# martinsbruveris/tensorflow-image-models

Hardware: NVIDIA H100
Metric: images/sec fwd bs=256 224px (higher is better)
Workload: dtype bf16

## Files before the change

tensorflow-image-models_b200/csrc/gemm_epilogue.cuh:

```cuda
#pragma once
#include "common.cuh"

namespace tfimm {

struct GemmParams {
  int M, N, K;
  const float* bias;
  const float* gamma;
  int act;
  int has_res;
  int act_post;
  void* c;
  const void* res;
  long ldc, ldr;
  const float* a_scale;
  int a_rows_per_img, a_imgs;
  int conv;
  int cv_cblocks;
  int cv_ks, cv_stride, cv_pad;
  int cv_pb, cv_ph, cv_pw;
  int cv_tiles_x, cv_tiles_y;
  int cv_B, cv_Ho, cv_Wo;
  int tk_imgs, m_out, glu;
  long img_c, img_r;
  const void* mul;
  long ld_mul, img_mul;
};

__device__ __forceinline__ long epilogue_row_offset(const GemmParams& p, int m_blk, int r, long ld) {
  if (p.conv == 0) {
    const long m = (long)m_blk * 128 + r;
    return m < p.M ? m * ld : -1;
  }
  const int tx = m_blk % p.cv_tiles_x, tyb = m_blk / p.cv_tiles_x;
  const int ty = tyb % p.cv_tiles_y, tb = tyb / p.cv_tiles_y;
  const int per_img = p.cv_ph * p.cv_pw;
  const int b = tb * p.cv_pb + r / per_img;
  const int y = ty * p.cv_ph + (r % per_img) / p.cv_pw;
  const int x = tx * p.cv_pw + r % p.cv_pw;
  if (b >= p.cv_B || y >= p.cv_Ho || x >= p.cv_Wo) return -1;
  return (((long)b * p.cv_Ho + y) * p.cv_Wo + x) * p.N;
}

template <int NP, bool kSharedRcp = false>
__device__ __forceinline__ void apply_act_pairs(uint64_t (&v)[NP], int act) {
  static_assert(NP % 2 == 0, "activations are evaluated on groups of four elements");
  switch (act) {
    case kActGelu:
#pragma unroll
      for (int j = 0; j < NP; j += 2) {
        gelu4<kSharedRcp>(v[j], v[j + 1]);
      }
      break;
    case kActSwish:
#pragma unroll
      for (int j = 0; j < NP; j += 2) {
        swish4<kSharedRcp>(v[j], v[j + 1]);
      }
      break;
    case kActNone:
      break;
    default:
#pragma unroll
      for (int j = 0; j < NP; ++j) {
        float a, b;
        unpack2(v[j], a, b);
        v[j] = pack2(apply_act<false>(a, act), apply_act<false>(b, act));
      }
      break;
  }
}

__device__ __forceinline__ uint64_t ld_pair_or(const float* __restrict__ vec, int n, int N, float neutral) {
  if (n + 1 < N) {
    const float2 f = __ldg(reinterpret_cast<const float2*>(vec + n));
    return pack2(f.x, f.y);
  }
  return pack2(n < N ? __ldg(vec + n) : neutral, neutral);
}

__device__ __forceinline__ uint64_t ld_out_pair(const float* p, bool two) {
  if (two) {
    const float2 f = *reinterpret_cast<const float2*>(p);
    return pack2(f.x, f.y);
  }
  return pack2(*p, 0.f);
}
__device__ __forceinline__ uint64_t ld_out_pair(const __nv_bfloat16* p, bool two) {
  if (two) {
    const float2 f = unpack_bf16x2(*reinterpret_cast<const uint32_t*>(p));
    return pack2(f.x, f.y);
  }
  return pack2(__bfloat162float(*p), 0.f);
}
__device__ __forceinline__ void st_out_pair(float* p, uint64_t v, bool two) {
  float a, b;
  unpack2(v, a, b);
  if (two) *reinterpret_cast<float2*>(p) = make_float2(a, b);
  else *p = a;
}
__device__ __forceinline__ void st_out_pair(__nv_bfloat16* p, uint64_t v, bool two) {
  float a, b;
  unpack2(v, a, b);
  if (two) *reinterpret_cast<uint32_t*>(p) = pack_bf16x2(a, b);
  else *p = __float2bfloat16_rn(a);
}

template <typename OutT, int BN>
__device__ __forceinline__ void epilogue_frag(const GemmParams& p, float (&acc)[BN / 2], int m_blk, int n_blk,
                                              int wg_row0) {
  constexpr int kRun = BN >= 256 ? 2 : 4;
  const int lane = threadIdx.x & 31, wq = (threadIdx.x >> 5) & 3;
  const int r = wg_row0 + wq * 16 + (lane >> 2);
  const long off_c[2] = {epilogue_row_offset(p, m_blk, r, p.ldc), epilogue_row_offset(p, m_blk, r + 8, p.ldc)};
  const long off_r[2] = {p.has_res ? epilogue_row_offset(p, m_blk, r, p.ldr) : -1,
                         p.has_res ? epilogue_row_offset(p, m_blk, r + 8, p.ldr) : -1};
  OutT* __restrict__ C = reinterpret_cast<OutT*>(p.c);
  const OutT* R = reinterpret_cast<const OutT*>(p.res);
#pragma unroll
  for (int g0 = 0; g0 < BN / 8; g0 += kRun) {
    if (n_blk * BN + g0 * 8 >= p.N) break;
    uint64_t b[kRun], s[kRun], res[kRun][2];
#pragma unroll
    for (int j = 0; j < kRun; ++j) {
      const int n = n_blk * BN + (g0 + j) * 8 + 2 * (lane & 3);
      const bool in = n < p.N, two = n + 1 < p.N;
      b[j] = p.bias != nullptr ? ld_pair_or(p.bias, n, p.N, 0.f) : 0;
      s[j] = p.gamma != nullptr ? ld_pair_or(p.gamma, n, p.N, 1.f) : 0;
#pragma unroll
      for (int h = 0; h < 2; ++h)
        res[j][h] = p.has_res && in && off_r[h] >= 0 ? ld_out_pair(R + off_r[h] + n, two) : 0;
    }
#pragma unroll
    for (int j = 0; j < kRun; ++j) {
      const int g = g0 + j;
      const int n = n_blk * BN + g * 8 + 2 * (lane & 3);
      if (n_blk * BN + g * 8 >= p.N) break;
      const bool in = n < p.N, two = n + 1 < p.N;
      uint64_t v[2] = {pack2(acc[4 * g + 0], acc[4 * g + 1]), pack2(acc[4 * g + 2], acc[4 * g + 3])};
      if (p.bias != nullptr) {
        v[0] = add2(v[0], b[j]);
        v[1] = add2(v[1], b[j]);
      }
      if (!p.act_post) apply_act_pairs(v, p.act);
      if (p.gamma != nullptr) {
        v[0] = mul2(v[0], s[j]);
        v[1] = mul2(v[1], s[j]);
      }
      if (p.has_res) {
#pragma unroll
        for (int h = 0; h < 2; ++h)
          if (in && off_r[h] >= 0) v[h] = add2(v[h], res[j][h]);
      }
      if (p.act_post) apply_act_pairs(v, p.act);
#pragma unroll
      for (int h = 0; h < 2; ++h)
        if (in && off_c[h] >= 0) st_out_pair(C + off_c[h] + n, v[h], two);
    }
  }
}

template <typename OutT>
constexpr int staged_chunk_cols() { return 128 / (int)sizeof(OutT); }
constexpr int kStagedBoxBytes = 64 * 128;

template <typename OutT>
__device__ __forceinline__ uint32_t staged_addr(uint32_t s_wg, int row, int col) {
  constexpr int kCols = staged_chunk_cols<OutT>();
  const uint32_t byte = (uint32_t)(col % kCols) * (uint32_t)sizeof(OutT);
  return s_wg + (uint32_t)(col / kCols) * kStagedBoxBytes + (uint32_t)row * 128u +
         ((((byte >> 4) ^ (uint32_t)(row & 7)) << 4) | (byte & 15u));
}
__device__ __forceinline__ uint64_t ld_staged_pair(const float*, uint32_t a) {
  float x, y;
  asm volatile("ld.shared.v2.f32 {%0, %1}, [%2];" : "=f"(x), "=f"(y) : "r"(a) : "memory");
  return pack2(x, y);
}
__device__ __forceinline__ uint64_t ld_staged_pair(const __nv_bfloat16*, uint32_t a) {
  uint32_t u;
  asm volatile("ld.shared.b32 %0, [%1];" : "=r"(u) : "r"(a) : "memory");
  const float2 f = unpack_bf16x2(u);
  return pack2(f.x, f.y);
}
__device__ __forceinline__ void st_staged_pair(float*, uint32_t a, uint64_t v) {
  float x, y;
  unpack2(v, x, y);
  asm volatile("st.shared.v2.f32 [%0], {%1, %2};" ::"r"(a), "f"(x), "f"(y) : "memory");
}
__device__ __forceinline__ void st_staged_pair(__nv_bfloat16*, uint32_t a, uint64_t v) {
  float x, y;
  unpack2(v, x, y);
  asm volatile("st.shared.b32 [%0], %1;" ::"r"(a), "r"(pack_bf16x2(x, y)) : "memory");
}

template <typename OutT, int BN>
__device__ __forceinline__ void epilogue_staged(const GemmParams& p, float (&acc)[BN / 2], int m_blk, int n_blk, int wg,
                                                uint32_t s_out, const float* s_bias, const float* s_gamma,
                                                uint32_t res_bar, const CUtensorMap* tmap_c) {
  constexpr int kCols = staged_chunk_cols<OutT>(), kChunks = BN / kCols;
  const int lane = threadIdx.x & 31, wq = (threadIdx.x >> 5) & 3;
  const int r = wq * 16 + (lane >> 2);
  const uint32_t s_wg = s_out + (uint32_t)(wg * kChunks * kStagedBoxBytes);
  OutT* const tag = nullptr;
  named_bar_sync<1>(256);
  if (p.has_res) mbar_wait(res_bar, 0);
#pragma unroll
  for (int g = 0; g < BN / 8; ++g) {
    const int c = g * 8 + 2 * (lane & 3);
    const uint32_t a0 = staged_addr<OutT>(s_wg, r, c), a1 = a0 + 8 * 128;
    uint64_t v[2] = {pack2(acc[4 * g + 0], acc[4 * g + 1]), pack2(acc[4 * g + 2], acc[4 * g + 3])};
    if (p.bias != nullptr) {
      const float2 b = *reinterpret_cast<const float2*>(s_bias + c);
      v[0] = add2(v[0], pack2(b.x, b.y));
      v[1] = add2(v[1], pack2(b.x, b.y));
    }
    if (!p.act_post) apply_act_pairs(v, p.act);
    if (p.gamma != nullptr) {
      const float2 s = *reinterpret_cast<const float2*>(s_gamma + c);
      v[0] = mul2(v[0], pack2(s.x, s.y));
      v[1] = mul2(v[1], pack2(s.x, s.y));
    }
    if (p.has_res) {
      v[0] = add2(v[0], ld_staged_pair(tag, a0));
      v[1] = add2(v[1], ld_staged_pair(tag, a1));
    }
    if (p.act_post) apply_act_pairs(v, p.act);
    st_staged_pair(tag, a0, v[0]);
    st_staged_pair(tag, a1, v[1]);
  }
  fence_proxy_async_smem();
  if (wg == 0) named_bar_sync<2>(128);
  else named_bar_sync<3>(128);
  const int row0 = m_blk * 128 + wg * 64;
  if ((threadIdx.x & 127) == 0 && row0 < p.M) {
#pragma unroll
    for (int ch = 0; ch < kChunks; ++ch) {
      const int col0 = n_blk * BN + ch * kCols;
      if (col0 < p.N) tma_store_2d(tmap_c, s_wg + (uint32_t)(ch * kStagedBoxBytes), col0, row0);
    }
    tma_store_commit();
    tma_store_wait_read<0>();
  }
}

template <typename OutT, int BN>
__device__ __forceinline__ void epilogue_token(const GemmParams& p, float (&acc)[BN / 2], int img, int m_blk, int n_blk,
                                               int wg_row0) {
  const int lane = threadIdx.x & 31, wq = (threadIdx.x >> 5) & 3;
  const int m0 = m_blk * 128 + wg_row0 + wq * 16 + (lane >> 2);
  const float b0 = p.bias != nullptr && m0 < p.M ? __ldg(p.bias + m0) : 0.f;
  const float b1 = p.bias != nullptr && m0 + 8 < p.M ? __ldg(p.bias + m0 + 8) : 0.f;
  const int rows[2] = {p.glu ? (m0 >> 4) * 8 + (m0 & 7) : m0, p.glu ? -1 : m0 + 8};
  OutT* __restrict__ C = reinterpret_cast<OutT*>(p.c) + (long)img * p.img_c;
  const OutT* R = reinterpret_cast<const OutT*>(p.res) + (long)img * p.img_r;
  const OutT* U = reinterpret_cast<const OutT*>(p.mul) + (long)img * p.img_mul;
#pragma unroll
  for (int g = 0; g < BN / 8; ++g) {
    const int n = n_blk * BN + g * 8 + 2 * (lane & 3);
    if (n_blk * BN + g * 8 >= p.N) break;
    const bool in = n < p.N, two = n + 1 < p.N;
    uint64_t v[2] = {pack2(acc[4 * g + 0] + b0, acc[4 * g + 1] + b0), pack2(acc[4 * g + 2] + b1, acc[4 * g + 3] + b1)};
    if (p.glu) {
      float x0, x1, g0, g1;
      unpack2(v[0], x0, x1);
      unpack2(v[1], g0, g1);
      v[0] = pack2(x0 * apply_act<false>(g0, p.act), x1 * apply_act<false>(g1, p.act));
    } else {
      apply_act_pairs(v, p.act);
    }
    if (p.gamma != nullptr) {
      const uint64_t s = ld_pair_or(p.gamma, n, p.N, 1.f);
      v[0] = mul2(v[0], s);
      v[1] = mul2(v[1], s);
    }
#pragma unroll
    for (int h = 0; h < 2; ++h) {
      const int row = rows[h];
      if (!in || row < 0 || row >= p.m_out) continue;
      if (p.mul != nullptr) v[h] = mul2(v[h], ld_out_pair(U + (long)row * p.ld_mul + n, two));
      if (p.has_res) v[h] = add2(v[h], ld_out_pair(R + (long)row * p.ldr + n, two));
      st_out_pair(C + (long)row * p.ldc + n, v[h], two);
    }
  }
}

template <typename OutT, int BN>
__device__ __forceinline__ void epilogue_glu_cols(const GemmParams& p, float (&acc)[BN / 2], int m_blk, int n_blk,
                                                  int wg_row0) {
  const int lane = threadIdx.x & 31, wq = (threadIdx.x >> 5) & 3;
  const int r = wg_row0 + wq * 16 + (lane >> 2);
  const long off_c[2] = {epilogue_row_offset(p, m_blk, r, p.ldc), epilogue_row_offset(p, m_blk, r + 8, p.ldc)};
  OutT* __restrict__ C = reinterpret_cast<OutT*>(p.c);
#pragma unroll
  for (int g = 0; g < BN / 8; ++g) {
    const int n = n_blk * BN + g * 8 + 2 * (lane & 3);
    if (n_blk * BN + g * 8 >= p.N) break;
    if (n >= p.N) continue;
    float bx = 0.f, bg = 0.f;
    if (p.bias != nullptr) {
      const float2 b = __ldg(reinterpret_cast<const float2*>(p.bias + n));
      bx = b.x; bg = b.y;
    }
#pragma unroll
    for (int h = 0; h < 2; ++h) {
      if (off_c[h] < 0) continue;
      const float x = acc[4 * g + 2 * h] + bx, gt = acc[4 * g + 2 * h + 1] + bg;
      const float y = x * apply_act<false>(gt, p.act);
      if constexpr (sizeof(OutT) == 2) C[off_c[h] + n / 2] = __float2bfloat16_rn(y);
      else C[off_c[h] + n / 2] = y;
    }
  }
}

}
```

tensorflow-image-models_b200/csrc/gemm_sm90.cu:

```cuda
#include <type_traits>

#include "gemm_epilogue.cuh"
#include "wgmma.cuh"

namespace tfimm {

namespace {

constexpr int kBlockM = 128;
constexpr int kRowBytes = 128;
constexpr int kConsumerThreads = 256;
constexpr int kProducerWarp = kConsumerThreads / 32;
constexpr int kNumGateWarps = 4;

enum ATransform : int {
  kANone = 0,
  kAGate = 1,
  kATf32 = 2,
};
enum GemmMode : int { kModeGemm = 0, kModeToken = 1, kModeGluCols = 2 };

template <int AX>
using OperandT = std::conditional_t<AX == kATf32, float, __nv_bfloat16>;
template <int AX>
constexpr int block_k() { return kRowBytes / (int)sizeof(OperandT<AX>); }
template <int AX>
constexpr int dtype_code() { return AX == kATf32 ? kF32 : kBF16; }

template <int BLOCK_N, typename OutT = float, bool STAGED = false>
struct GemmCfg {
  static constexpr int kABytes = kBlockM * kRowBytes;
  static constexpr int kBBytes = BLOCK_N * kRowBytes;
  static constexpr int kStageBytes = kABytes + kBBytes;
  static constexpr int kStages = STAGED && BLOCK_N == 64 ? 3 : 4;
  static constexpr int kOutBytes = STAGED ? kBlockM * BLOCK_N * (int)sizeof(OutT) : 0;
  static constexpr int kVecBytes = STAGED ? 2 * BLOCK_N * 4 : 0;
  static constexpr int kNumBarriers = 3 * kStages + 1;
  static constexpr int kSmemBytes =
      kStages * kStageBytes + kOutBytes + kVecBytes + kNumBarriers * 8 + 1024 ;
  static_assert(!STAGED || BLOCK_N <= 128, "the staged epilogue's tile does not fit next to a 256-wide ring");
};

template <bool kMN>
__device__ __forceinline__ uint64_t gmma_desc_b(uint32_t smem_addr) {
  if constexpr (kMN) return gmma_desc_mn_sw128(smem_addr);
  else return gmma_desc_k_sw128(smem_addr);
}
template <bool kMN>
constexpr int kDescStepB = kMN ? 128 : 2;

template <int BLOCK_N, int AX>
constexpr int gemm_threads() { return kConsumerThreads + 32 + (AX != kANone ? 32 * kNumGateWarps : 0); }

template <int BLOCK_N, typename OutT, int AX = kANone, int MODE = kModeGemm, bool STAGED = false>
__global__ void __launch_bounds__(gemm_threads<BLOCK_N, AX>(), (BLOCK_N == 64 && AX == kANone) ? 2 : 1)
gemm_wgmma_kernel(const __grid_constant__ CUtensorMap tmap_a, const __grid_constant__ CUtensorMap tmap_b,
                  const __grid_constant__ CUtensorMap tmap_c, const __grid_constant__ CUtensorMap tmap_r,
                  const GemmParams p) {
  static_assert(!STAGED || (AX == kANone && MODE == kModeGemm), "staged epilogue: plain bf16 GEMM only");
  using Cfg = GemmCfg<BLOCK_N, OutT, STAGED>;
  constexpr int kStages = Cfg::kStages;
  constexpr int kBlockK = block_k<AX>();

  extern __shared__ uint8_t smem_raw[];
  const uint32_t smem_base = (smem_u32(smem_raw) + 1023u) & ~1023u;
  const uint32_t smem_tiles = smem_base;
  const uint32_t smem_out = smem_base + kStages * Cfg::kStageBytes;
  const uint32_t smem_vec = smem_out + Cfg::kOutBytes;
  const uint32_t smem_bars = smem_vec + Cfg::kVecBytes;
  auto full_bar = [&](int s) { return smem_bars + 8u * s; };
  auto empty_bar = [&](int s) { return smem_bars + 8u * (kStages + s); };
  auto ready_bar = [&](int s) { return smem_bars + 8u * (2 * kStages + s); };
  const uint32_t res_bar = smem_bars + 8u * (3 * kStages);
  float* const s_bias = reinterpret_cast<float*>(smem_raw + (smem_vec - smem_u32(smem_raw)));
  float* const s_gamma = s_bias + BLOCK_N;

  const int warp_idx = threadIdx.x >> 5;
  const int lane = threadIdx.x & 31;

  if (warp_idx == kProducerWarp && lane == 0) {
    prefetch_tmap(&tmap_a);
    prefetch_tmap(&tmap_b);
    if constexpr (STAGED) {
      prefetch_tmap(&tmap_c);
      if (p.has_res) prefetch_tmap(&tmap_r);
      mbar_init(res_bar, 1);
    }
    for (int s = 0; s < kStages; ++s) {
      mbar_init(full_bar(s), 1);
      mbar_init(empty_bar(s), 2);
      mbar_init(ready_bar(s), 1);
    }
    fence_mbar_init();
  }
  __syncthreads();

  const int num_n_tiles = (p.N + BLOCK_N - 1) / BLOCK_N;
  int m_blk, n_blk, img = 0;
  if constexpr (MODE == kModeToken) {
    const int img_tiles = ((p.M + kBlockM - 1) / kBlockM) * num_n_tiles;
    img = (int)blockIdx.x / img_tiles;
    const int tile = (int)blockIdx.x - img * img_tiles;
    m_blk = tile / num_n_tiles; n_blk = tile % num_n_tiles;
  } else {
    m_blk = blockIdx.x / num_n_tiles; n_blk = blockIdx.x % num_n_tiles;
  }
  const int num_k_blocks = (p.K + kBlockK - 1) / kBlockK;

  if (warp_idx == kProducerWarp) {
    if (lane == 0) {
      int stage = 0;
      uint32_t phase = 0;
      for (int kb = 0; kb < num_k_blocks; ++kb) {
        mbar_wait(empty_bar(stage), phase ^ 1u);
        const uint32_t sa = smem_tiles + stage * Cfg::kStageBytes;
        const uint32_t sb = sa + Cfg::kABytes;
        mbar_expect_tx(full_bar(stage), Cfg::kStageBytes);
        if (STAGED || p.conv == 0) {
          tma_load_2d(sa, &tmap_a, full_bar(stage), kb * kBlockK, m_blk * kBlockM);
        } else {
          const int tap = kb / p.cv_cblocks, cb = kb - tap * p.cv_cblocks;
          const int ky = tap / p.cv_ks, kx = tap - ky * p.cv_ks;
          const int tx = m_blk % p.cv_tiles_x, tyb = m_blk / p.cv_tiles_x;
          const int ty = tyb % p.cv_tiles_y, tb = tyb / p.cv_tiles_y;
          tma_load_4d(sa, &tmap_a, full_bar(stage), cb * kBlockK, tx * p.cv_pw * p.cv_stride + kx - p.cv_pad,
                      ty * p.cv_ph * p.cv_stride + ky - p.cv_pad, tb * p.cv_pb);
        }
        if constexpr (MODE == kModeToken) {
#pragma unroll
          for (int i = 0; i < BLOCK_N / 64; ++i)
            tma_load_3d(sb + i * 8192, &tmap_b, full_bar(stage), n_blk * BLOCK_N + i * 64, kb * kBlockK, img);
        } else {
          tma_load_2d(sb, &tmap_b, full_bar(stage), kb * kBlockK, n_blk * BLOCK_N);
        }
        if constexpr (STAGED) {
          if (kb == 0 && p.has_res) {
            constexpr int kCols = staged_chunk_cols<OutT>(), kChunks = BLOCK_N / kCols;
            const int row0 = m_blk * kBlockM, col0 = n_blk * BLOCK_N;
            const int rows = p.M - row0 > 64 ? 2 : 1, chunks = min(kChunks, (p.N - col0 + kCols - 1) / kCols);
            mbar_expect_tx(res_bar, (uint32_t)(rows * chunks * kStagedBoxBytes));
            for (int h = 0; h < rows; ++h)
              for (int ch = 0; ch < chunks; ++ch)
                tma_load_2d(smem_out + (uint32_t)((h * kChunks + ch) * kStagedBoxBytes), &tmap_r, res_bar,
                            col0 + ch * kCols, row0 + 64 * h);
          }
        }
        if (++stage == kStages) { stage = 0; phase ^= 1u; }
      }
    }
  } else if (AX != kANone && warp_idx > kProducerWarp) {
    const int wt = warp_idx - kProducerWarp - 1;
    const int c = lane & 7, r0 = lane >> 3;
    auto load_gate = [&](int img, int k0, float4& ga, float4& gb) {
      const float* g = p.a_scale + (long)img * p.K + k0;
      ga = __ldg(reinterpret_cast<const float4*>(g));
      gb = __ldg(reinterpret_cast<const float4*>(g + 4));
    };
    int img0 = 0;
    long bound0 = 0;
    if constexpr (AX == kAGate) {
      const long row_first = (long)m_blk * kBlockM + r0;
      long im0 = row_first / p.a_rows_per_img;
      im0 = im0 < p.a_imgs ? im0 : p.a_imgs - 1;
      img0 = (int)im0;
      bound0 = (im0 + 1) * p.a_rows_per_img - (long)m_blk * kBlockM;
    }
    int stage = 0, turn = 0;
    uint32_t phase = 0;
    for (int kb = 0; kb < num_k_blocks; ++kb) {
      if (turn == wt) {
        if constexpr (AX == kATf32) {
          mbar_wait(full_bar(stage), phase);
          const uint32_t sa = smem_tiles + stage * Cfg::kStageBytes;
#pragma unroll 1
          for (int b8 = 0; b8 < 4; ++b8) {
            uint4 u[8];
#pragma unroll
            for (int i = 0; i < 8; ++i) {
              const int r = r0 + 4 * (8 * b8 + i);
              asm volatile("ld.shared.v4.u32 {%0, %1, %2, %3}, [%4];"
                           : "=r"(u[i].x), "=r"(u[i].y), "=r"(u[i].z), "=r"(u[i].w)
                           : "r"(sa + (uint32_t)(r * 128 + (c << 4))));
            }
#pragma unroll
            for (int i = 0; i < 8; ++i) {
              const int r = r0 + 4 * (8 * b8 + i);
              asm volatile("st.shared.v4.u32 [%0], {%1, %2, %3, %4};" ::"r"(sa + (uint32_t)(r * 128 + (c << 4))),
                           "r"(tf32_rna(__uint_as_float(u[i].x))), "r"(tf32_rna(__uint_as_float(u[i].y))),
                           "r"(tf32_rna(__uint_as_float(u[i].z))), "r"(tf32_rna(__uint_as_float(u[i].w)))
                           : "memory");
            }
          }
        } else {
          const int k0 = kb * kBlockK + c * 8;
          const bool valid = k0 < p.K;
          float4 ga = make_float4(0.f, 0.f, 0.f, 0.f), gb = ga;
          if (valid) load_gate(img0, k0, ga, gb);
          mbar_wait(full_bar(stage), phase);
          if (valid) {
            const uint32_t sa = smem_tiles + stage * Cfg::kStageBytes;
            int cur = img0;
            long bound = bound0;
#pragma unroll 1
            for (int b8 = 0; b8 < 4; ++b8) {
              uint4 u[8];
#pragma unroll
              for (int i = 0; i < 8; ++i) {
                const int r = r0 + 4 * (8 * b8 + i);
                asm volatile("ld.shared.v4.u32 {%0, %1, %2, %3}, [%4];"
                             : "=r"(u[i].x), "=r"(u[i].y), "=r"(u[i].z), "=r"(u[i].w)
                             : "r"(sa + (uint32_t)(r * 128 + ((c ^ (r & 7)) << 4))));
              }
#pragma unroll
              for (int i = 0; i < 8; ++i) {
                const int r = r0 + 4 * (8 * b8 + i);
                if (r >= bound && cur < p.a_imgs - 1) {
                  do { ++cur; bound += p.a_rows_per_img; } while (r >= bound && cur < p.a_imgs - 1);
                  load_gate(cur, k0, ga, gb);
                }
                const float2 x0 = unpack_bf16x2(u[i].x), x1 = unpack_bf16x2(u[i].y), x2 = unpack_bf16x2(u[i].z),
                             x3 = unpack_bf16x2(u[i].w);
                const uint32_t o0 = pack_bf16x2(x0.x * ga.x, x0.y * ga.y), o1 = pack_bf16x2(x1.x * ga.z, x1.y * ga.w);
                const uint32_t o2 = pack_bf16x2(x2.x * gb.x, x2.y * gb.y), o3 = pack_bf16x2(x3.x * gb.z, x3.y * gb.w);
                asm volatile("st.shared.v4.u32 [%0], {%1, %2, %3, %4};"
                             ::"r"(sa + (uint32_t)(r * 128 + ((c ^ (r & 7)) << 4))), "r"(o0), "r"(o1), "r"(o2), "r"(o3)
                             : "memory");
              }
            }
          }
        }
        fence_proxy_async_smem();
        __syncwarp();
        if (lane == 0) mbar_arrive(ready_bar(stage));
      }
      turn = turn + 1 == kNumGateWarps ? 0 : turn + 1;
      if (++stage == kStages) { stage = 0; phase ^= 1u; }
    }
  } else if (warp_idx < kProducerWarp) {
    const int wg = warp_idx >> 2;
    const bool releaser = (threadIdx.x & 127) == 0;
    if constexpr (STAGED) {
      const int t = threadIdx.x, n = n_blk * BLOCK_N + (t % BLOCK_N);
      if (t < BLOCK_N && p.bias != nullptr) s_bias[t] = n < p.N ? __ldg(p.bias + n) : 0.f;
      if (t >= BLOCK_N && t < 2 * BLOCK_N && p.gamma != nullptr) s_gamma[t - BLOCK_N] = n < p.N ? __ldg(p.gamma + n) : 1.f;
    }
    float acc[BLOCK_N / 2];
#pragma unroll
    for (int i = 0; i < BLOCK_N / 2; ++i) acc[i] = 0.f;
    int stage = 0, prev = 0;
    uint32_t phase = 0;
    for (int kb = 0; kb < num_k_blocks; ++kb) {
      mbar_wait(AX != kANone ? ready_bar(stage) : full_bar(stage), phase);
      const uint32_t sa = smem_tiles + stage * Cfg::kStageBytes;
      const uint64_t da = gmma_desc_k_sw128(sa + (uint32_t)wg * (64 * 128));
      const uint64_t db = gmma_desc_b<MODE == kModeToken>(sa + Cfg::kABytes);
      wgmma_fence();
#pragma unroll
      for (int k = 0; k < 4; ++k) {
        if constexpr (AX == kATf32)
          wgmma_ss_tf32<BLOCK_N>(acc, da + (uint64_t)(2 * k), db + (uint64_t)(2 * k), (uint32_t)((kb | k) != 0));
        else
          wgmma_ss<BLOCK_N, MODE == kModeToken>(acc, da + (uint64_t)(2 * k), db + (uint64_t)(kDescStepB<MODE == kModeToken> * k),
                                                (uint32_t)((kb | k) != 0));
      }
      wgmma_commit();
      wgmma_wait<1>();
      if (kb > 0 && releaser) mbar_arrive(empty_bar(prev));
      prev = stage;
      if (++stage == kStages) { stage = 0; phase ^= 1u; }
    }
    wgmma_wait<0>();
    if (releaser) mbar_arrive(empty_bar(prev));
    if constexpr (MODE == kModeToken) epilogue_token<OutT, BLOCK_N>(p, acc, img, m_blk, n_blk, wg * 64);
    else if constexpr (MODE == kModeGluCols) epilogue_glu_cols<OutT, BLOCK_N>(p, acc, m_blk, n_blk, wg * 64);
    else if constexpr (STAGED)
      epilogue_staged<OutT, BLOCK_N>(p, acc, m_blk, n_blk, wg, smem_out, s_bias, s_gamma, res_bar, &tmap_c);
    else epilogue_frag<OutT, BLOCK_N>(p, acc, m_blk, n_blk, wg * 64);
  }
}

int check_out(const void* C, long ldc, const void* residual, long ldr, int esize) {
  TFIMM_CHECK_ARG((reinterpret_cast<uintptr_t>(C) & 15u) == 0 && (ldc * esize) % 16 == 0,
                  "gemm: C must be 16-byte aligned with a row stride of a multiple of 16 bytes");
  TFIMM_CHECK_ARG(residual == nullptr || ((reinterpret_cast<uintptr_t>(residual) & 15u) == 0 && (ldr * esize) % 16 == 0),
                  "gemm: residual must be 16-byte aligned with a row stride of a multiple of 16 bytes");
  return kOk;
}

template <int BLOCK_N, typename OutT, int AX, int MODE, bool STAGED = false>
int launch_wgmma(const CUtensorMap& ta, const CUtensorMap& tb, const GemmParams& p, const char* what,
                 cudaStream_t stream, const CUtensorMap& tc = CUtensorMap{}, const CUtensorMap& tr = CUtensorMap{}) {
  using Cfg = GemmCfg<BLOCK_N, OutT, STAGED>;
  auto kernel = gemm_wgmma_kernel<BLOCK_N, OutT, AX, MODE, STAGED>;
  static std::atomic<unsigned long long> attr_devs{0};
  TFIMM_CUDA_OK(set_max_dynamic_smem(kernel, Cfg::kSmemBytes, attr_devs));
  const long imgs = MODE == kModeToken ? p.tk_imgs : 1;
  const long tiles = imgs * ((p.M + kBlockM - 1) / kBlockM) * ((p.N + BLOCK_N - 1) / BLOCK_N);
  kernel<<<(unsigned)tiles, gemm_threads<BLOCK_N, AX>(), Cfg::kSmemBytes, stream>>>(ta, tb, tc, tr, p);
  TFIMM_LAUNCH_OK(what);
  return kOk;
}

template <int kMaxN, typename F>
int with_block_n(int bn, const char* unsupported_fmt, F&& launch) {
  if constexpr (kMaxN >= 256) {
    if (bn == 256) return launch(std::integral_constant<int, 256>{});
  }
  if (bn == 128) return launch(std::integral_constant<int, 128>{});
  if (bn == 64) return launch(std::integral_constant<int, 64>{});
  set_last_error(unsupported_fmt, bn);
  return kInvalidArgument;
}

template <int BLOCK_N, typename OutT, int AX = kANone, int MODE = kModeGemm>
int launch_gemm(const void* A, int lda, const void* W, int ldw, const void* residual, int ldr, void* C, int ldc,
                GemmParams p, cudaStream_t stream) {
  const int M = p.M, N = p.N, K = p.K;
  constexpr int kBlockK = block_k<AX>();
  CUtensorMap ta, tb;
  int st;
  if ((st = check_out(C, ldc, residual, ldr, (int)sizeof(OutT))) != kOk) return st;
  if ((st = make_tmap_2d(&ta, A, dtype_code<AX>(), M, K, lda, kBlockM, kBlockK, "A")) != kOk) return st;
  if ((st = make_tmap_2d(&tb, W, dtype_code<AX>(), N, K, ldw, BLOCK_N, kBlockK, "W")) != kOk) return st;
  p.c = C; p.res = residual; p.ldc = ldc; p.ldr = ldr;
  constexpr bool kStaged = AX == kANone && MODE == kModeGemm && BLOCK_N <= 128;
  if constexpr (kStaged) {
    if ((long)N * (long)sizeof(OutT) % 16 != 0)
      return launch_wgmma<BLOCK_N, OutT, AX, MODE>(ta, tb, p, "gemm_wgmma_kernel (bf16)", stream);
    constexpr int es = (int)sizeof(OutT), dt = es == 2 ? kBF16 : kF32;
    CUtensorMap tc, tr{};
    if ((st = make_tmap_2d(&tc, C, dt, M, N, ldc, 64, staged_chunk_cols<OutT>(), "C")) != kOk) return st;
    if (residual != nullptr &&
        (st = make_tmap_2d(&tr, residual, dt, M, N, ldr, 64, staged_chunk_cols<OutT>(), "residual")) != kOk)
      return st;
    return launch_wgmma<BLOCK_N, OutT, AX, MODE, true>(ta, tb, p, "gemm_wgmma_kernel (bf16)", stream, tc, tr);
  }
  return launch_wgmma<BLOCK_N, OutT, AX, MODE>(
      ta, tb, p,
      AX == kATf32 ? "gemm_wgmma_kernel (tf32)"
                   : (MODE == kModeGluCols ? "gemm_wgmma_kernel (bf16 glu)" : "gemm_wgmma_kernel (bf16)"),
      stream);
}

template <int BLOCK_N, typename OutT>
int launch_token(const void* Wt, int ldw, const void* X, long ldx, long img_x, GemmParams p, cudaStream_t stream) {
  CUtensorMap ta, tb;
  int st;
  if ((st = check_out(p.c, p.ldc, p.res, p.ldr, (int)sizeof(OutT))) != kOk) return st;
  if ((st = make_tmap_2d(&ta, Wt, kBF16, p.M, p.K, ldw, kBlockM, 64, "token Wt")) != kOk) return st;
  {
    const uint64_t dims[3] = {(uint64_t)p.N, (uint64_t)p.K, (uint64_t)p.tk_imgs};
    const uint64_t strides[2] = {(uint64_t)ldx * 2, (uint64_t)img_x * 2};
    const uint32_t box[3] = {64u, 64u, 1u};
    if ((st = make_tmap(&tb, X, kBF16, 3, dims, strides, box, "token X")) != kOk) return st;
  }
  return launch_wgmma<BLOCK_N, OutT, kANone, kModeToken>(ta, tb, p, "gemm_wgmma_kernel (bf16 token mixing)", stream);
}

template <int BLOCK_N, typename OutT, int AX = kANone>
int launch_conv(const void* x, const void* W, int ldw, const void* residual, void* out, int B, int H, int Wd, int C,
                int Ho, int Wo, GemmParams p, cudaStream_t stream) {
  constexpr int kBlockK = block_k<AX>();
  constexpr uint64_t es = sizeof(OperandT<AX>);
  const int N = p.N, s = p.cv_stride;
  CUtensorMap ta, tb;
  int st;
  if ((st = check_out(out, N, residual, N, (int)sizeof(OutT))) != kOk) return st;
  {
    const uint64_t dims[4] = {(uint64_t)C, (uint64_t)Wd, (uint64_t)H, (uint64_t)B};
    const uint64_t strides[3] = {(uint64_t)C * es, (uint64_t)Wd * C * es, (uint64_t)H * Wd * C * es};
    const uint32_t box[4] = {(uint32_t)kBlockK, (uint32_t)(p.cv_pw * s), (uint32_t)(p.cv_ph * s), (uint32_t)p.cv_pb};
    const uint32_t estr[4] = {1u, (uint32_t)s, (uint32_t)s, 1u};
    if ((st = make_tmap(&ta, x, dtype_code<AX>(), 4, dims, strides, box, "conv input", 128, estr)) != kOk) return st;
  }
  if ((st = make_tmap_2d(&tb, W, dtype_code<AX>(), N, p.K, ldw, BLOCK_N, kBlockK, "conv weights")) != kOk) return st;
  p.c = out; p.res = residual; p.ldc = N; p.ldr = N;
  p.cv_B = B; p.cv_Ho = Ho; p.cv_Wo = Wo;
  return launch_wgmma<BLOCK_N, OutT, AX, kModeGemm>(
      ta, tb, p,
      AX == kATf32 ? "gemm_wgmma_kernel (tf32 implicit convolution)" : "gemm_wgmma_kernel (bf16 implicit convolution)",
      stream);
}

int pick_block_n(int M, int N) {
  const int sms = sm_count() > 0 ? sm_count() : 132;
  const int mt = (M + kBlockM - 1) / kBlockM;
  int best = 256;
  double best_cost = 1e30;
  for (int bn : {256, 128, 64}) {
    const int nt = (N + bn - 1) / bn;
    const long tiles = (long)mt * nt;
    const int slots = bn == 64 ? 2 * sms : sms;
    const long waves = (tiles + slots - 1) / slots;
    const double cost = (double)waves * (bn == 64 ? 2 * bn : bn) * (bn == 256 ? 1.0 : (bn == 128 ? 1.04 : 1.10));
    if (cost < best_cost) { best_cost = cost; best = bn; }
  }
  return best;
}

int pick_block_n_bf16(int M, int N, int K) {
  constexpr double kEpilogueK = 926.0, kPairWidth = 184.0;
  const int sms = sm_count() > 0 ? sm_count() : 132;
  const long mt = (M + kBlockM - 1) / kBlockM;
  const long waves128 = (mt * ((N + 127) / 128) + sms - 1) / sms;
  const long waves64 = (mt * ((N + 63) / 64) + 2 * sms - 1) / (2 * sms);
  return (double)waves64 * kPairWidth * K < (double)waves128 * 128.0 * (K + kEpilogueK) ? 64 : 128;
}

}

int gemm_bf16_skinny(const void* A, int lda, const void* W, int ldw, const float* bias, const void* residual, int ldr,
                     void* C, int ldc, int M, int N, int K, int act, cudaStream_t stream, const float* gate = nullptr,
                     int rows_per_img = 1, int imgs = 1);

int conv_setup(GemmParams& p, const float* bias, const void* residual, int B, int H, int Wd, int C, int N, int ks,
               int stride, int pad, int act, int act_post, int cblock, int& Ho, int& Wo) {
  TFIMM_CHECK_ARG(B > 0 && H > 0 && Wd > 0 && C > 0 && C % cblock == 0, "conv: C must be a multiple of %d (got %d)",
                  cblock, C);
  TFIMM_CHECK_ARG(ks >= 1 && ks <= 7 && (stride == 1 || stride == 2) && pad >= 0 && pad < ks, "conv: bad geometry");
  TFIMM_CHECK_ARG(N > 0 && N % 8 == 0, "conv: N must be a multiple of 8 (got %d)", N);
  TFIMM_CHECK_ARG(bias == nullptr || (reinterpret_cast<uintptr_t>(bias) & 15u) == 0, "conv: bias must be 16-byte aligned");
  Ho = (H + 2 * pad - ks) / stride + 1;
  Wo = (Wd + 2 * pad - ks) / stride + 1;
  TFIMM_CHECK_ARG(Ho > 0 && Wo > 0, "conv: empty output");
  p = GemmParams{};
  p.N = N; p.K = ks * ks * C;
  p.bias = bias; p.act = act; p.has_res = residual != nullptr ? 1 : 0; p.act_post = act_post;
  p.conv = 1; p.cv_cblocks = C / cblock; p.cv_ks = ks; p.cv_stride = stride; p.cv_pad = pad;
  if (Wo > 8) { p.cv_pb = 1; p.cv_ph = 8; p.cv_pw = 16; }
  else { p.cv_pb = 2; p.cv_ph = 8; p.cv_pw = 8; }
  p.cv_tiles_x = (Wo + p.cv_pw - 1) / p.cv_pw;
  p.cv_tiles_y = (Ho + p.cv_ph - 1) / p.cv_ph;
  const int tiles_b = (B + p.cv_pb - 1) / p.cv_pb;
  p.M = tiles_b * p.cv_tiles_y * p.cv_tiles_x * kBlockM;
  return kOk;
}

}

using namespace tfimm;

extern "C" {

int tfimm_b200_gemm_bf16(const void* A, int lda, const void* W, int ldw, const float* bias, const float* gamma,
                         const void* residual, int ldr, void* C, int ldc, int M, int N, int K, int act, int act_post,
                         int out_dtype, int force_block_n, void* s) {
  const cudaStream_t stream = as_stream(s);
  TFIMM_CHECK_ARG(M > 0 && N > 0 && K > 0, "gemm: M, N, K must be positive (got %d %d %d)", M, N, K);
  TFIMM_CHECK_ARG(out_dtype == kBF16 || out_dtype == kF32, "gemm: out_dtype must be bf16 or f32");
  TFIMM_CHECK_ARG(K % 8 == 0, "gemm: K must be a multiple of 8 (got %d)", K);
  TFIMM_CHECK_ARG(bias == nullptr || (reinterpret_cast<uintptr_t>(bias) & 15u) == 0, "gemm: bias must be 16-byte aligned");
  TFIMM_CHECK_ARG(gamma == nullptr || (reinterpret_cast<uintptr_t>(gamma) & 15u) == 0, "gemm: gamma must be 16-byte aligned");
  if (force_block_n == 0 && K <= 64 && out_dtype == kBF16 && gamma == nullptr && act_post == 0) {
    const int st = gemm_bf16_skinny(A, lda, W, ldw, bias, residual, ldr, C, ldc, M, N, K, act, stream);
    if (st != kUnsupported) return st;
  }
  GemmParams p{};
  p.M = M; p.N = N; p.K = K;
  p.bias = bias; p.gamma = gamma; p.act = act; p.has_res = residual != nullptr ? 1 : 0; p.act_post = act_post;
  const int bn = force_block_n == 2 ? 256 : (force_block_n > 0 ? force_block_n : pick_block_n_bf16(M, N, K));
  return with_block_n<256>(bn, "gemm: unsupported block_n %d", [&](auto n) {
    constexpr int BN = decltype(n)::value;
    return out_dtype == kBF16 ? launch_gemm<BN, __nv_bfloat16>(A, lda, W, ldw, residual, ldr, C, ldc, p, stream)
                              : launch_gemm<BN, float>(A, lda, W, ldw, residual, ldr, C, ldc, p, stream);
  });
}

int tfimm_b200_gemm_bf16_gated(const void* A, int lda, const float* gate, int rows_per_img, int imgs, const void* W,
                               int ldw, const float* bias, const void* residual, int ldr, void* C, int ldc, int M,
                               int N, int K, int act, void* s) {
  const cudaStream_t stream = as_stream(s);
  TFIMM_CHECK_ARG(M > 0 && N > 0 && K > 0 && K % 8 == 0, "gemm_gated: need K %% 8 == 0 (got M=%d N=%d K=%d)", M, N, K);
  TFIMM_CHECK_ARG(gate != nullptr && rows_per_img > 0 && imgs > 0 && (reinterpret_cast<uintptr_t>(gate) & 15u) == 0,
                  "gemm_gated: gate [imgs][K] fp32, 16-byte aligned");
  TFIMM_CHECK_ARG(bias == nullptr || (reinterpret_cast<uintptr_t>(bias) & 15u) == 0, "gemm_gated: bias must be 16-byte aligned");
  if (K <= 64) {
    const int st = gemm_bf16_skinny(A, lda, W, ldw, bias, residual, ldr, C, ldc, M, N, K, act, stream, gate, rows_per_img,
                                    imgs);
    if (st != kUnsupported) return st;
  }
  GemmParams p{};
  p.M = M; p.N = N; p.K = K;
  p.bias = bias; p.act = act; p.has_res = residual != nullptr ? 1 : 0;
  p.a_scale = gate; p.a_rows_per_img = rows_per_img; p.a_imgs = imgs;
  return with_block_n<128>(pick_block_n(M, N) == 64 ? 64 : 128, "gemm_gated: unsupported block_n %d", [&](auto n) {
    return launch_gemm<decltype(n)::value, __nv_bfloat16, kAGate>(A, lda, W, ldw, residual, ldr, C, ldc, p, stream);
  });
}

int tfimm_b200_conv_bf16(const void* x, const void* W, int ldw, const float* bias, const void* residual, void* out,
                         int B, int H, int Wd, int C, int N, int ks, int stride, int pad, int act, int act_post,
                         int out_dtype, void* s) {
  const cudaStream_t stream = as_stream(s);
  TFIMM_CHECK_ARG(out_dtype == kBF16 || out_dtype == kF32, "conv: out_dtype must be bf16 or f32");
  GemmParams p;
  int Ho, Wo, st;
  if ((st = conv_setup(p, bias, residual, B, H, Wd, C, N, ks, stride, pad, act, act_post, 64, Ho, Wo)) != kOk)
    return st;
  return with_block_n<256>(N >= 256 ? 256 : (N >= 128 ? 128 : 64), "conv: unsupported block_n %d", [&](auto n) {
    constexpr int BN = decltype(n)::value;
    return out_dtype == kBF16 ? launch_conv<BN, __nv_bfloat16>(x, W, ldw, residual, out, B, H, Wd, C, Ho, Wo, p, stream)
                              : launch_conv<BN, float>(x, W, ldw, residual, out, B, H, Wd, C, Ho, Wo, p, stream);
  });
}

int tfimm_b200_gemm_tf32(const float* A, int lda, const float* W, int ldw, const float* bias, const float* gamma,
                         const float* residual, int ldr, float* C, int ldc, int M, int N, int K, int act, int act_post,
                         int force_block_n, void* s) {
  const cudaStream_t stream = as_stream(s);
  TFIMM_CHECK_ARG(M > 0 && N > 0 && K > 0, "gemm_tf32: M, N, K must be positive (got %d %d %d)", M, N, K);
  TFIMM_CHECK_ARG(K % 4 == 0, "gemm_tf32: K must be a multiple of 4 (got %d)", K);
  TFIMM_CHECK_ARG(bias == nullptr || (reinterpret_cast<uintptr_t>(bias) & 15u) == 0, "gemm_tf32: bias must be 16-byte aligned");
  TFIMM_CHECK_ARG(gamma == nullptr || (reinterpret_cast<uintptr_t>(gamma) & 15u) == 0,
                  "gemm_tf32: gamma must be 16-byte aligned");
  GemmParams p{};
  p.M = M; p.N = N; p.K = K;
  p.bias = bias; p.gamma = gamma; p.act = act; p.has_res = residual != nullptr ? 1 : 0; p.act_post = act_post;
  const int bn = force_block_n == 2 ? 128 : (force_block_n > 0 ? force_block_n : (pick_block_n(M, N) == 64 ? 64 : 128));
  return with_block_n<128>(bn, "gemm_tf32: unsupported block_n %d (64 or 128)", [&](auto n) {
    return launch_gemm<decltype(n)::value, float, kATf32>(A, lda, W, ldw, residual, ldr, C, ldc, p, stream);
  });
}

int tfimm_b200_conv_tf32(const float* x, const float* W, int ldw, const float* bias, const float* residual, float* out,
                         int B, int H, int Wd, int C, int N, int ks, int stride, int pad, int act, int act_post,
                         void* s) {
  const cudaStream_t stream = as_stream(s);
  GemmParams p;
  int Ho, Wo, st;
  if ((st = conv_setup(p, bias, residual, B, H, Wd, C, N, ks, stride, pad, act, act_post, 32, Ho, Wo)) != kOk)
    return st;
  return with_block_n<128>(N >= 128 ? 128 : 64, "conv: unsupported block_n %d", [&](auto n) {
    return launch_conv<decltype(n)::value, float, kATf32>(x, W, ldw, residual, out, B, H, Wd, C, Ho, Wo, p, stream);
  });
}

int tfimm_b200_token_gemm_bf16(const void* Wt, int ldw, const void* X, long ldx, long img_x, const float* bias,
                               const float* gamma, const void* residual, long ldr, long img_r, const void* mul,
                               long ld_mul, long img_mul, void* out, long ldc, long img_c, int imgs, int M, int N,
                               int K, int m_out, int act, int glu, int out_dtype, int force_block_n, void* s) {
  const cudaStream_t stream = as_stream(s);
  TFIMM_CHECK_ARG(imgs > 0 && M > 0 && N > 0 && K > 0 && m_out > 0, "token_gemm: empty shape (imgs %d M %d N %d K %d)",
                  imgs, M, N, K);
  TFIMM_CHECK_ARG(out_dtype == kBF16 || out_dtype == kF32, "token_gemm: out_dtype must be bf16 or f32");
  TFIMM_CHECK_ARG(ldw % 8 == 0 && ldw >= K && ldx % 8 == 0 && img_x % 8 == 0 && ldx >= N,
                  "token_gemm: Wt / X strides must be multiples of 8 elements");
  TFIMM_CHECK_ARG(glu ? (M % 16 == 0 && m_out <= M / 2) : m_out <= M, "token_gemm: m_out %d does not fit M %d (glu %d)",
                  m_out, M, glu);
  TFIMM_CHECK_ARG(N % 2 == 0 && (gamma == nullptr || (reinterpret_cast<uintptr_t>(gamma) & 7u) == 0),
                  "token_gemm: N must be even and gamma 8-byte aligned");
  const int es = out_dtype == kBF16 ? 2 : 4;
  TFIMM_CHECK_ARG(mul == nullptr || ((reinterpret_cast<uintptr_t>(mul) & 15u) == 0 && (ld_mul * es) % 16 == 0 &&
                                     (img_mul * es) % 16 == 0),
                  "token_gemm: mul must be 16-byte aligned with strides of multiples of 16 bytes");
  TFIMM_CHECK_ARG((img_c * es) % 16 == 0 && (residual == nullptr || (img_r * es) % 16 == 0),
                  "token_gemm: image strides must be multiples of 16 bytes");
  GemmParams p{};
  p.M = M; p.N = N; p.K = K;
  p.bias = bias; p.gamma = gamma; p.act = act; p.has_res = residual != nullptr ? 1 : 0;
  p.c = out; p.res = residual; p.ldc = ldc; p.ldr = ldr;
  p.tk_imgs = imgs; p.m_out = m_out; p.glu = glu; p.img_c = img_c; p.img_r = img_r;
  p.mul = mul; p.ld_mul = ld_mul; p.img_mul = img_mul;
  const int bn = force_block_n > 0 ? force_block_n : pick_block_n(imgs * ((M + kBlockM - 1) / kBlockM) * kBlockM, N);
  return with_block_n<256>(bn, "token_gemm: unsupported block_n %d", [&](auto n) {
    constexpr int BN = decltype(n)::value;
    return out_dtype == kBF16 ? launch_token<BN, __nv_bfloat16>(Wt, ldw, X, ldx, img_x, p, stream)
                              : launch_token<BN, float>(Wt, ldw, X, ldx, img_x, p, stream);
  });
}

int tfimm_b200_gemm_glu_bf16(const void* A, int lda, const void* W, int ldw, const float* bias, void* C, int ldc, int M,
                             int N, int K, int act, int force_block_n, void* s) {
  const cudaStream_t stream = as_stream(s);
  TFIMM_CHECK_ARG(M > 0 && N > 0 && K > 0 && K % 8 == 0 && N % 2 == 0,
                  "gemm_glu: need K %% 8 == 0 and an even N (got M=%d N=%d K=%d)", M, N, K);
  TFIMM_CHECK_ARG(bias == nullptr || (reinterpret_cast<uintptr_t>(bias) & 7u) == 0, "gemm_glu: bias must be 8-byte aligned");
  GemmParams p{};
  p.M = M; p.N = N; p.K = K;
  p.bias = bias; p.act = act;
  const int bn = force_block_n > 0 ? force_block_n : pick_block_n(M, N);
  return with_block_n<256>(bn, "gemm_glu: unsupported block_n %d", [&](auto n) {
    return launch_gemm<decltype(n)::value, __nv_bfloat16, kANone, kModeGluCols>(A, lda, W, ldw, nullptr, 0, C, ldc, p,
                                                                               stream);
  });
}

}
```

Measured before the change: 10010.

## Add persistent 256-wide staged GEMM kernel with overlapped epilogue and residual prefetch

Adds a persistent bf16 GEMM kernel with 256-column tiles that loops over output tiles on a grid sized to the SM count. It double-buffers bias and gamma vectors, prefetches residual tiles via TMA midway through the K loop, and splits the staged epilogue into spans so TMA stores overlap the next tile's mainloop. The staged epilogue is also specialized on the activation type at compile time. The heuristic routes large GEMMs (N>256 with enough tiles) to this path, trading smaller tiles and wave quantization for larger tiles and more shared-memory pressure.

```diff
diff --git a/tensorflow-image-models_b200/csrc/gemm_epilogue.cuh b/tensorflow-image-models_b200/csrc/gemm_epilogue.cuh
--- a/tensorflow-image-models_b200/csrc/gemm_epilogue.cuh
+++ b/tensorflow-image-models_b200/csrc/gemm_epilogue.cuh
@@ -193,28 +193,24 @@
   asm volatile("st.shared.b32 [%0], %1;" ::"r"(a), "r"(pack_bf16x2(x, y)) : "memory");
 }
 
-template <typename OutT, int BN>
-__device__ __forceinline__ void epilogue_staged(const GemmParams& p, float (&acc)[BN / 2], int m_blk, int n_blk, int wg,
-                                                uint32_t s_out, const float* s_bias, const float* s_gamma,
-                                                uint32_t res_bar, const CUtensorMap* tmap_c) {
-  constexpr int kCols = staged_chunk_cols<OutT>(), kChunks = BN / kCols;
+template <typename OutT, int BN, int kFirst, int kSpan, int kAct>
+__device__ __forceinline__ void staged_apply_act(const GemmParams& p, float (&acc)[BN / 2], uint32_t s_wg,
+                                                 const float* s_bias, const float* s_gamma) {
+  const int act = kAct >= 0 ? kAct : p.act;
   const int lane = threadIdx.x & 31, wq = (threadIdx.x >> 5) & 3;
   const int r = wq * 16 + (lane >> 2);
-  const uint32_t s_wg = s_out + (uint32_t)(wg * kChunks * kStagedBoxBytes);
   OutT* const tag = nullptr;
-  named_bar_sync<1>(256);
-  if (p.has_res) mbar_wait(res_bar, 0);
-#pragma unroll
-  for (int g = 0; g < BN / 8; ++g) {
+#pragma unroll
+  for (int g = kFirst / 8; g < (kFirst + kSpan) / 8; ++g) {
     const int c = g * 8 + 2 * (lane & 3);
-    const uint32_t a0 = staged_addr<OutT>(s_wg, r, c), a1 = a0 + 8 * 128;
+    const uint32_t a0 = staged_addr<OutT>(s_wg, r, c - kFirst), a1 = a0 + 8 * 128;
     uint64_t v[2] = {pack2(acc[4 * g + 0], acc[4 * g + 1]), pack2(acc[4 * g + 2], acc[4 * g + 3])};
     if (p.bias != nullptr) {
       const float2 b = *reinterpret_cast<const float2*>(s_bias + c);
       v[0] = add2(v[0], pack2(b.x, b.y));
       v[1] = add2(v[1], pack2(b.x, b.y));
     }
-    if (!p.act_post) apply_act_pairs(v, p.act);
+    if (!p.act_post) apply_act_pairs(v, act);
     if (p.gamma != nullptr) {
       const float2 s = *reinterpret_cast<const float2*>(s_gamma + c);
       v[0] = mul2(v[0], pack2(s.x, s.y));
@@ -224,21 +220,52 @@
       v[0] = add2(v[0], ld_staged_pair(tag, a0));
       v[1] = add2(v[1], ld_staged_pair(tag, a1));
     }
-    if (p.act_post) apply_act_pairs(v, p.act);
+    if (p.act_post) apply_act_pairs(v, act);
     st_staged_pair(tag, a0, v[0]);
     st_staged_pair(tag, a1, v[1]);
   }
-  fence_proxy_async_smem();
+}
+
+template <typename OutT, int BN, int kFirst, int kSpan>
+__device__ __forceinline__ void staged_apply(const GemmParams& p, float (&acc)[BN / 2], uint32_t s_wg,
+                                             const float* s_bias, const float* s_gamma) {
+  switch (p.act) {
+    case kActNone: staged_apply_act<OutT, BN, kFirst, kSpan, kActNone>(p, acc, s_wg, s_bias, s_gamma); break;
+    case kActGelu: staged_apply_act<OutT, BN, kFirst, kSpan, kActGelu>(p, acc, s_wg, s_bias, s_gamma); break;
+    case kActSwish: staged_apply_act<OutT, BN, kFirst, kSpan, kActSwish>(p, acc, s_wg, s_bias, s_gamma); break;
+    default: staged_apply_act<OutT, BN, kFirst, kSpan, -1>(p, acc, s_wg, s_bias, s_gamma); break;
+  }
+}
+
+__device__ __forceinline__ void warpgroup_bar_sync(int wg) {
   if (wg == 0) named_bar_sync<2>(128);
   else named_bar_sync<3>(128);
+}
+
+template <typename OutT, int kChunks>
+__device__ __forceinline__ void staged_store(const GemmParams& p, const CUtensorMap* tmap_c, uint32_t s_wg, int row0,
+                                             int col0) {
+  constexpr int kCols = staged_chunk_cols<OutT>();
+#pragma unroll
+  for (int ch = 0; ch < kChunks; ++ch)
+    if (col0 + ch * kCols < p.N) tma_store_2d(tmap_c, s_wg + (uint32_t)(ch * kStagedBoxBytes), col0 + ch * kCols, row0);
+  tma_store_commit();
+}
+
+template <typename OutT, int BN>
+__device__ __forceinline__ void epilogue_staged(const GemmParams& p, float (&acc)[BN / 2], int m_blk, int n_blk, int wg,
+                                                uint32_t s_out, const float* s_bias, const float* s_gamma,
+                                                uint32_t res_bar, const CUtensorMap* tmap_c) {
+  constexpr int kChunks = BN / staged_chunk_cols<OutT>();
+  const uint32_t s_wg = s_out + (uint32_t)(wg * kChunks * kStagedBoxBytes);
+  named_bar_sync<1>(256);
+  if (p.has_res) mbar_wait(res_bar, 0);
+  staged_apply<OutT, BN, 0, BN>(p, acc, s_wg, s_bias, s_gamma);
+  fence_proxy_async_smem();
+  warpgroup_bar_sync(wg);
   const int row0 = m_blk * 128 + wg * 64;
   if ((threadIdx.x & 127) == 0 && row0 < p.M) {
-#pragma unroll
-    for (int ch = 0; ch < kChunks; ++ch) {
-      const int col0 = n_blk * BN + ch * kCols;
-      if (col0 < p.N) tma_store_2d(tmap_c, s_wg + (uint32_t)(ch * kStagedBoxBytes), col0, row0);
-    }
-    tma_store_commit();
+    staged_store<OutT, kChunks>(p, tmap_c, s_wg, row0, n_blk * BN);
     tma_store_wait_read<0>();
   }
 }
diff --git a/tensorflow-image-models_b200/csrc/gemm_sm90.cu b/tensorflow-image-models_b200/csrc/gemm_sm90.cu
--- a/tensorflow-image-models_b200/csrc/gemm_sm90.cu
+++ b/tensorflow-image-models_b200/csrc/gemm_sm90.cu
@@ -279,6 +279,152 @@
   }
 }
 
+struct PersistentCfg {
+  static constexpr int kBlockN = 256;
+  static constexpr int kABytes = kBlockM * kRowBytes;
+  static constexpr int kStageBytes = kABytes + kBlockN * kRowBytes;
+  static constexpr int kStages = 3;
+  static constexpr int kBoxes = 4;
+  static constexpr int kOutBytes = 2 * kBoxes * kStagedBoxBytes;
+  static constexpr int kVecBytes = 2 * 2 * kBlockN * 4;
+  static constexpr int kNumBarriers = 2 * kStages + 2;
+  static constexpr int kSmemBytes = kStages * kStageBytes + kOutBytes + kVecBytes + kNumBarriers * 8 + 1024;
+};
+
+template <typename OutT>
+__global__ void __launch_bounds__(kConsumerThreads + 32, 1)
+gemm_persistent_kernel(const __grid_constant__ CUtensorMap tmap_a, const __grid_constant__ CUtensorMap tmap_b,
+                       const __grid_constant__ CUtensorMap tmap_c, const __grid_constant__ CUtensorMap tmap_r,
+                       const GemmParams p) {
+  using Cfg = PersistentCfg;
+  constexpr int BN = Cfg::kBlockN, kStages = Cfg::kStages, kBlockK = 64;
+  constexpr int kCols = staged_chunk_cols<OutT>(), kSpan = Cfg::kBoxes * kCols;
+
+  extern __shared__ uint8_t smem_raw[];
+  const uint32_t smem_tiles = (smem_u32(smem_raw) + 1023u) & ~1023u;
+  const uint32_t smem_out = smem_tiles + kStages * Cfg::kStageBytes;
+  const uint32_t smem_vec = smem_out + Cfg::kOutBytes;
+  const uint32_t smem_bars = smem_vec + Cfg::kVecBytes;
+  auto full_bar = [&](int s) { return smem_bars + 8u * s; };
+  auto empty_bar = [&](int s) { return smem_bars + 8u * (kStages + s); };
+  float* const s_vec = reinterpret_cast<float*>(smem_raw + (smem_vec - smem_u32(smem_raw)));
+
+  const int warp_idx = threadIdx.x >> 5;
+  const int lane = threadIdx.x & 31;
+  if (warp_idx == kProducerWarp && lane == 0) {
+    prefetch_tmap(&tmap_a);
+    prefetch_tmap(&tmap_b);
+    prefetch_tmap(&tmap_c);
+    if (p.has_res) prefetch_tmap(&tmap_r);
+    for (int s = 0; s < kStages; ++s) {
+      mbar_init(full_bar(s), 1);
+      mbar_init(empty_bar(s), 2);
+    }
+    mbar_init(smem_bars + 8u * (2 * kStages), 1);
+    mbar_init(smem_bars + 8u * (2 * kStages + 1), 1);
+    fence_mbar_init();
+  }
+  __syncthreads();
+
+  const int num_n_tiles = (p.N + BN - 1) / BN;
+  const int tiles = ((p.M + kBlockM - 1) / kBlockM) * num_n_tiles;
+  const int num_k_blocks = (p.K + kBlockK - 1) / kBlockK;
+
+  if (warp_idx == kProducerWarp) {
+    if (threadIdx.x == kProducerWarp * 32) {
+      int stage = 0;
+      uint32_t phase = 0;
+      for (int t = blockIdx.x; t < tiles; t += gridDim.x) {
+        const int m_blk = t / num_n_tiles, n_blk = t % num_n_tiles;
+        for (int kb = 0; kb < num_k_blocks; ++kb) {
+          mbar_wait(empty_bar(stage), phase ^ 1u);
+          const uint32_t sa = smem_tiles + stage * Cfg::kStageBytes;
+          mbar_expect_tx(full_bar(stage), Cfg::kStageBytes);
+          tma_load_2d(sa, &tmap_a, full_bar(stage), kb * kBlockK, m_blk * kBlockM);
+          tma_load_2d(sa + Cfg::kABytes, &tmap_b, full_bar(stage), kb * kBlockK, n_blk * BN);
+          if (++stage == kStages) { stage = 0; phase ^= 1u; }
+        }
+      }
+    }
+    return;
+  }
+
+  const int wg = warp_idx >> 2;
+  const bool leader = (threadIdx.x & 127) == 0;
+  const uint32_t s_wg = smem_out + (uint32_t)(wg * Cfg::kBoxes * kStagedBoxBytes);
+  const uint32_t res_bar = smem_bars + 8u * (2 * kStages + wg);
+  int stage = 0, prev = 0, buf = 0;
+  uint32_t phase = 0, res_phase = 0;
+  for (int t = blockIdx.x; t < tiles; t += gridDim.x, buf ^= 1) {
+    const int m_blk = t / num_n_tiles, n_blk = t % num_n_tiles;
+    const int row0 = m_blk * kBlockM + wg * 64;
+    auto has_res_span = [&](int h) { return p.has_res && row0 < p.M && n_blk * BN + h * kSpan < p.N; };
+    auto load_res_span = [&](int h) {
+      const int col0 = n_blk * BN + h * kSpan, chunks = min(Cfg::kBoxes, (p.N - col0 + kCols - 1) / kCols);
+      mbar_expect_tx(res_bar, (uint32_t)(chunks * kStagedBoxBytes));
+      for (int ch = 0; ch < chunks; ++ch)
+        tma_load_2d(s_wg + (uint32_t)(ch * kStagedBoxBytes), &tmap_r, res_bar, col0 + ch * kCols, row0);
+    };
+    float* const s_bias = s_vec + buf * 2 * BN;
+    float* const s_gamma = s_bias + BN;
+    const int n_own = n_blk * BN + threadIdx.x;
+    const float bias_own = p.bias != nullptr && n_own < p.N ? __ldg(p.bias + n_own) : 0.f;
+    const float gamma_own = p.gamma != nullptr && n_own < p.N ? __ldg(p.gamma + n_own) : 1.f;
+    float acc[BN / 2];
+#pragma unroll
+    for (int i = 0; i < BN / 2; ++i) acc[i] = 0.f;
+    for (int kb = 0; kb < num_k_blocks; ++kb) {
+      mbar_wait(full_bar(stage), phase);
+      const uint32_t sa = smem_tiles + stage * Cfg::kStageBytes;
+      const uint64_t da = gmma_desc_k_sw128(sa + (uint32_t)wg * (64 * 128));
+      const uint64_t db = gmma_desc_k_sw128(sa + Cfg::kABytes);
+      wgmma_fence();
+#pragma unroll
+      for (int k = 0; k < 4; ++k)
+        wgmma_ss<BN, false>(acc, da + (uint64_t)(2 * k), db + (uint64_t)(2 * k), (uint32_t)((kb | k) != 0));
+      wgmma_commit();
+      if (kb == 0) {
+        s_bias[threadIdx.x] = bias_own;
+        s_gamma[threadIdx.x] = gamma_own;
+      }
+      if (kb == num_k_blocks / 2 && leader) {
+        tma_store_wait_read<0>();
+        if (has_res_span(0)) load_res_span(0);
+      }
+      wgmma_wait<1>();
+      if (kb > 0 && leader) mbar_arrive(empty_bar(prev));
+      prev = stage;
+      if (++stage == kStages) { stage = 0; phase ^= 1u; }
+    }
+    wgmma_wait<0>();
+    if (leader) mbar_arrive(empty_bar(prev));
+
+    named_bar_sync<1>(256);
+    auto span = [&](auto h_const) {
+      constexpr int h = decltype(h_const)::value;
+      if (n_blk * BN + h * kSpan >= p.N) return;
+      if constexpr (h > 0) {
+        if (leader) {
+          tma_store_wait_read<0>();
+          if (has_res_span(h)) load_res_span(h);
+        }
+        warpgroup_bar_sync(wg);
+      }
+      if (has_res_span(h)) {
+        mbar_wait(res_bar, res_phase);
+        res_phase ^= 1u;
+      }
+      staged_apply<OutT, BN, h * kSpan, kSpan>(p, acc, s_wg, s_bias, s_gamma);
+      fence_proxy_async_smem();
+      warpgroup_bar_sync(wg);
+      if (leader && row0 < p.M) staged_store<OutT, Cfg::kBoxes>(p, &tmap_c, s_wg, row0, n_blk * BN + h * kSpan);
+    };
+    span(std::integral_constant<int, 0>{});
+    if constexpr (kSpan < BN) span(std::integral_constant<int, 1>{});
+  }
+  if (leader) tma_store_wait_read<0>();
+}
+
 int check_out(const void* C, long ldc, const void* residual, long ldr, int esize) {
   TFIMM_CHECK_ARG((reinterpret_cast<uintptr_t>(C) & 15u) == 0 && (ldc * esize) % 16 == 0,
                   "gemm: C must be 16-byte aligned with a row stride of a multiple of 16 bytes");
@@ -312,9 +458,25 @@
   return kInvalidArgument;
 }
 
-template <int BLOCK_N, typename OutT, int AX = kANone, int MODE = kModeGemm>
+template <typename OutT>
+int launch_persistent(const CUtensorMap& ta, const CUtensorMap& tb, const CUtensorMap& tc, const CUtensorMap& tr,
+                      const GemmParams& p, cudaStream_t stream) {
+  using Cfg = PersistentCfg;
+  auto kernel = gemm_persistent_kernel<OutT>;
+  static std::atomic<unsigned long long> attr_devs{0};
+  TFIMM_CUDA_OK(set_max_dynamic_smem(kernel, Cfg::kSmemBytes, attr_devs));
+  const long tiles = (long)((p.M + kBlockM - 1) / kBlockM) * ((p.N + Cfg::kBlockN - 1) / Cfg::kBlockN);
+  const int grid = (int)std::min<long>(tiles, sm_count());
+  kernel<<<grid, kConsumerThreads + 32, Cfg::kSmemBytes, stream>>>(ta, tb, tc, tr, p);
+  TFIMM_LAUNCH_OK("gemm_persistent_kernel (bf16)");
+  return kOk;
+}
+
+template <int BLOCK_N, typename OutT, int AX = kANone, int MODE = kModeGemm, bool PERSISTENT = false>
 int launch_gemm(const void* A, int lda, const void* W, int ldw, const void* residual, int ldr, void* C, int ldc,
                 GemmParams p, cudaStream_t stream) {
+  static_assert(!PERSISTENT || (BLOCK_N == PersistentCfg::kBlockN && AX == kANone && MODE == kModeGemm),
+                "the persistent instance is the plain bf16 GEMM at 256 columns");
   const int M = p.M, N = p.N, K = p.K;
   constexpr int kBlockK = block_k<AX>();
   CUtensorMap ta, tb;
@@ -323,7 +485,7 @@
   if ((st = make_tmap_2d(&ta, A, dtype_code<AX>(), M, K, lda, kBlockM, kBlockK, "A")) != kOk) return st;
   if ((st = make_tmap_2d(&tb, W, dtype_code<AX>(), N, K, ldw, BLOCK_N, kBlockK, "W")) != kOk) return st;
   p.c = C; p.res = residual; p.ldc = ldc; p.ldr = ldr;
-  constexpr bool kStaged = AX == kANone && MODE == kModeGemm && BLOCK_N <= 128;
+  constexpr bool kStaged = AX == kANone && MODE == kModeGemm && (BLOCK_N <= 128 || PERSISTENT);
   if constexpr (kStaged) {
     if ((long)N * (long)sizeof(OutT) % 16 != 0)
       return launch_wgmma<BLOCK_N, OutT, AX, MODE>(ta, tb, p, "gemm_wgmma_kernel (bf16)", stream);
@@ -333,7 +495,8 @@
     if (residual != nullptr &&
         (st = make_tmap_2d(&tr, residual, dt, M, N, ldr, 64, staged_chunk_cols<OutT>(), "residual")) != kOk)
       return st;
-    return launch_wgmma<BLOCK_N, OutT, AX, MODE, true>(ta, tb, p, "gemm_wgmma_kernel (bf16)", stream, tc, tr);
+    if constexpr (PERSISTENT) return launch_persistent<OutT>(ta, tb, tc, tr, p, stream);
+    else return launch_wgmma<BLOCK_N, OutT, AX, MODE, true>(ta, tb, p, "gemm_wgmma_kernel (bf16)", stream, tc, tr);
   }
   return launch_wgmma<BLOCK_N, OutT, AX, MODE>(
       ta, tb, p,
@@ -398,10 +561,13 @@
   return best;
 }
 
-int pick_block_n_bf16(int M, int N, int K) {
+constexpr int kPersistent = 1;
+
+int pick_block_n_bf16(int M, int N, int K, int out_dtype) {
   constexpr double kEpilogueK = 926.0, kPairWidth = 184.0;
   const int sms = sm_count() > 0 ? sm_count() : 132;
   const long mt = (M + kBlockM - 1) / kBlockM;
+  if (N > 256 && (out_dtype == kF32 || N % 8 == 0) && mt * ((N + 255) / 256) >= sms) return kPersistent;
   const long waves128 = (mt * ((N + 127) / 128) + sms - 1) / sms;
   const long waves64 = (mt * ((N + 63) / 64) + 2 * sms - 1) / (2 * sms);
   return (double)waves64 * kPairWidth * K < (double)waves128 * 128.0 * (K + kEpilogueK) ? 64 : 128;
@@ -458,7 +624,12 @@
   GemmParams p{};
   p.M = M; p.N = N; p.K = K;
   p.bias = bias; p.gamma = gamma; p.act = act; p.has_res = residual != nullptr ? 1 : 0; p.act_post = act_post;
-  const int bn = force_block_n == 2 ? 256 : (force_block_n > 0 ? force_block_n : pick_block_n_bf16(M, N, K));
+  const int bn =
+      force_block_n == 2 ? 256 : (force_block_n > 0 ? force_block_n : pick_block_n_bf16(M, N, K, out_dtype));
+  if (bn == kPersistent)
+    return out_dtype == kBF16
+               ? launch_gemm<256, __nv_bfloat16, kANone, kModeGemm, true>(A, lda, W, ldw, residual, ldr, C, ldc, p, stream)
+               : launch_gemm<256, float, kANone, kModeGemm, true>(A, lda, W, ldw, residual, ldr, C, ldc, p, stream);
   return with_block_n<256>(bn, "gemm: unsupported block_n %d", [&](auto n) {
     constexpr int BN = decltype(n)::value;
     return out_dtype == kBF16 ? launch_gemm<BN, __nv_bfloat16>(A, lda, W, ldw, residual, ldr, C, ldc, p, stream)
```

New measurement: 11750, median of 6. 17.3% higher.
